# edshkim98/DiffusionIQT

Hardware: AMD Instinct MI355X
Metric: 3D patches/sec (32³, 1ch) — sample steps/sec x batch (one U-Net eval per patch and step: DDPM ancestral; EDM Heun in `edm` / `unet3d_edm`, train-steps/sec in `train`) (higher is better)
Workload: dtype f32; 1 GPU; C2: SRUnet256 dim=64 mults=(1,2,4) 32^3 1ch, batch 8/GPU, DDPM ancestral sampler step (1 U-Net eval = 186.06 GFLOP/patch); global_batch=8, patch=32^3, parallelism=dp1

## Files before the change

### diffusioniqt_amd/_lib.py

```python
import ctypes
import os

import torch
from ctypes import c_int, c_float, c_size_t, c_void_p, c_longlong, c_char_p

_HERE = os.path.dirname(os.path.abspath(__file__))
LIB_PATH = os.environ.get("DIQT_LIB") or os.path.join(_HERE, "csrc", "libdiqt_hip.so")

P, I, F, Z, L = c_void_p, c_int, c_float, c_size_t, c_longlong

PROTOTYPES = {
    "diqt_version": (I, []),
    "diqt_last_error": (c_char_p, []),
    "diqt_census_enable": (I, [I]),
    "diqt_census_count": (L, [c_char_p]),
    "diqt_get_last_launch": (c_char_p, []),
    "diqt_conv_packed_elems": (Z, [I, I, I, I, I]),
    "diqt_conv_packed_wino_elems": (Z, [I, I, I, I, I]),
    "diqt_conv_pack_weight": (I, [P, P, I, I, I, I, I, I, P]),
    "diqt_conv3d_fwd": (I, [P, P, P, P, P] + [I] * 15 + [P]),
    "diqt_conv3d_fwd_workspace_bytes": (Z, [I] * 15),
    "diqt_conv3d_fwd_ws": (I, [P, P, P, P, P, P, Z] + [I] * 15 + [P]),
    "diqt_conv3d_lds_bytes": (L, [I] * 12),
    "diqt_trilinear_up_fwd": (I, [P, P, I, I, I, I, I, I, P]),
# ... 198 lines not shown
    "diqt_conv_packed_split16_elems": (Z, [I, I, I, I, I]),
    "diqt_conv_pack_weight_split16": (I, [P, P, P, I, I, I, I, I, P]),
    "diqt_conv3d_fwd_split16_supported": (I, [I] * 15),
    "diqt_conv3d_fwd_gn_split16_supported": (I, [I] * 16),
    "diqt_conv3d_fwd_split16_stats_blocks": (I, [I] * 15),
    "diqt_conv3d_fwd_split16_variant": (I, [I] * 15),
    "diqt_conv3d_fwd_split16": (I, [P, P, P, P, P, P, P] + [I] * 15 + [P]),
    "diqt_conv3d_fwd_gn_split16": (I, [P, P, P, P, P, P, P, P, I] + [I] * 15 + [P]),
    "diqt_set_conv_split16_fill_tile": (I, [I]),
    "diqt_conv3d_fwd_split16_fill_supported": (I, [I] * 15),
    "diqt_conv3d_fwd_gn_split16_fill_supported": (I, [I] * 16),
    "diqt_conv3d_fwd_split16_fill_stats_blocks": (I, [I] * 15),
    "diqt_conv3d_fwd_split16_fill_variant": (I, [I] * 15),
    "diqt_conv3d_fwd_split16_fill": (I, [P, P, P, P, P, P, P] + [I] * 15 + [P]),
    "diqt_conv3d_fwd_gn_split16_fill": (I, [P, P, P, P, P, P, P, P, I] + [I] * 15 + [P]),
}

_lib = None


def load():
    global _lib
    if _lib is not None:
        return _lib
    if not os.path.exists(LIB_PATH):
        raise RuntimeError(
            f"diffusioniqt_amd: {LIB_PATH} is missing — build it with `python -c 'import __graft_entry__ as g; "
            f"g.build()'` or `bash diffusioniqt_amd/csrc/build.sh`. There is no CPU fallback.")
    lib = ctypes.CDLL(LIB_PATH)
    for name, (res, args) in PROTOTYPES.items():
# ... 75 lines not shown
```

### diffusioniqt_amd/csrc/conv_f9h_kernel.h

```cpp
#pragma once
#include "common.h"
#include "conv_f9h.h"

namespace diqt {
namespace h9 {

typedef float f32x16 __attribute__((ext_vector_type(16)));
typedef float f32x4v __attribute__((ext_vector_type(4)));
typedef unsigned u32x4 __attribute__((ext_vector_type(4)));
typedef unsigned u32x2 __attribute__((ext_vector_type(2)));
typedef _Float16 f16x8 __attribute__((ext_vector_type(8)));
typedef __bf16 bf16x8 __attribute__((ext_vector_type(8)));
typedef __attribute__((address_space(3))) void lds_void;

constexpr unsigned OOB = 0x80000000u;
constexpr int CK = 32, ROWB = 64;
constexpr int PD = 9;
constexpr int SCRW = 32 * 144;
constexpr int BIASB = 256;

#ifndef DIQT_F9H_STAMP
#define DIQT_F9H_STAMP(it, c, point)
#endif

// ... 495 lines not shown
    lds += BIASB;
    hipError_t e = hipFuncSetAttribute(reinterpret_cast<const void*>(kern), hipFuncAttributeMaxDynamicSharedMemorySize, (int)lds);
    DIQT_REQUIRE(e == hipSuccess, DIQT_E_LAUNCH, "conv3d_fwd_split16(v9h): hipFuncSetAttribute: %s", hipGetErrorString(e));
    hipLaunchKernelGGL(kern, dim3(grid), dim3(256), lds, (hipStream_t)stream, x, wp, bias, residual, y, g);
    return check_launch("conv3d_fwd_split16(v9h)");
}

int launch_b(const void* x, const unsigned short* wp, const float* bias, const float* residual, void* y, const H9Geom& g, size_t lds,
             unsigned grid, int bf16, bool yHalf, void* stream);
int launch_c(const void* x, const unsigned short* wp, const float* bias, const float* residual, void* y, const H9Geom& g, size_t lds,
             unsigned grid, int bf16, bool yHalf, void* stream);
int launch_split(const void* x, const unsigned short* wp, const float* bias, const float* residual, void* y, const H9Geom& g, size_t lds,
                 unsigned grid, void* stream);
int launch_split_b(const void* x, const unsigned short* wp, const float* bias, const float* residual, void* y, const H9Geom& g, size_t lds,
                   unsigned grid, void* stream);

}
}
```

### diffusioniqt_amd/csrc/conv_split16.hip

```cpp
#include "conv_f9h_kernel.h"
#include <atomic>

namespace diqt {

constexpr int S16_CG = 16;
constexpr float S16_MAX = 65504.f, S16_SCALE = 2048.f;

__device__ __forceinline__ float s16_clamp(float v) { return v > S16_MAX ? S16_MAX : (v < -S16_MAX ? -S16_MAX : v); }

__device__ __forceinline__ void s16_split(float v, _Float16& head, _Float16& tail) {
    head = (_Float16)s16_clamp(v);
    tail = (_Float16)s16_clamp((v - (float)head) * S16_SCALE);
}

__global__ __launch_bounds__(256) void conv_pack_weight_split16_kernel(const float* __restrict__ w, unsigned short* __restrict__ packed,
                                                                       int* __restrict__ refused, int Cout, int Cin, int T, int CoutPad,
                                                                       size_t total) {
    for (size_t i = blockIdx.x * (size_t)blockDim.x + threadIdx.x; i < total; i += (size_t)gridDim.x * blockDim.x) {
        const int k = (int)(i % h9::CK);
        size_t r = i / h9::CK;
        const int o = (int)(r % CoutPad);
        r /= CoutPad;
        const int tap = (int)(r % T);
        const int in = (int)(r / T) * S16_CG + (k & (S16_CG - 1));
// ... 31 lines not shown
            s16_split(v[e], h, t);
            head[e] = h; tail[e] = t;
        }
        unsigned short* row = y + vox * (size_t)(2 * C) + (size_t)(c8 >> 1) * 32u + (c8 & 1u) * 8u;
        *reinterpret_cast<h8*>(row) = head;
        *reinterpret_cast<h8*>(row + S16_CG) = tail;
    }
}

namespace h9 {

int launch_split(const void* x, const unsigned short* wp, const float* bias, const float* residual, void* y, const H9Geom& g, size_t lds,
                 unsigned grid, void* stream) {
    if (g.variant == 6) return launch_split_cfg<H9S_333_256>(x, wp, bias, residual, y, g, lds, grid, stream);
    if (g.variant == 7 || g.variant == 8) return launch_split_b(x, wp, bias, residual, y, g, lds, grid, stream);
    set_error("conv3d_fwd_split16(v9h): no variant %d", g.variant);
    return DIQT_E_UNSUPPORTED;
}

}
}

using namespace diqt;

extern "C" int diqt_set_conv_f9h_mode(int mode);

static bool split16_plan(H9Geom& g, size_t& lds, unsigned& grid, int B, int D, int H, int W, int Cin, int Cout, int kd, int kh, int kw, int pd,
                         int ph, int pw, int epd, int eph, int epw) {
    if (Cin <= 0 || Cin % S16_CG != 0 || Cin > (1 << 20)) return false;
    if (!f9h_plan(g, lds, grid, B, D, H, W, 2 * Cin, Cout, kd, kh, kw, pd, ph, pw, epd, eph, epw, false, true)) return false;
// ... 17 lines not shown
        if (forced && v != forced) continue;
        H9Geom t; size_t l; unsigned gr;
        if (!f9h_plan(t, l, gr, B, D, H, W, 2 * Cin, Cout, kd, kh, kw, pd, ph, pw, epd, eph, epw, false, true, v)) continue;
        g = t; lds = l; grid = gr; have = true;
        if ((long long)t.MT * t.nNt >= 256) break;
    }
    if (!have) return false;
    if (!lifted) {
        if ((long long)g.MT * g.nNt < 128) return false;
        if (g.variant == 8 && (long long)g.MT * g.nNt < 256 && Cin > 128) return false;
        if ((unsigned long long)B * g.Do * g.Ho * g.Wo * (unsigned long long)Cin * (unsigned long long)Cout < (1ull << 25)) return false;
    }
    return true;
}

static bool split16_any_plan(bool fill, H9Geom& g, size_t& lds, unsigned& grid, int B, int D, int H, int W, int Cin, int Cout, int kd, int kh,
                             int kw, int pd, int ph, int pw, int epd, int eph, int epw) {
    return fill ? split16_fill_plan(g, lds, grid, B, D, H, W, Cin, Cout, kd, kh, kw, pd, ph, pw, epd, eph, epw)
                : split16_plan(g, lds, grid, B, D, H, W, Cin, Cout, kd, kh, kw, pd, ph, pw, epd, eph, epw);
}

static bool split16_act_ok(int act) { return act == 0 || act == DIQT_ACT_MISH || act == DIQT_ACT_SILU || act == DIQT_ACT_GELU; }

extern "C" size_t diqt_conv_packed_split16_elems(int Cout, int Cin, int kd, int kh, int kw) {
    if (Cout <= 0 || Cin <= 0 || kd <= 0 || kh <= 0 || kw <= 0) return 0;
    return (size_t)((Cin + S16_CG - 1) / S16_CG) * kd * kh * kw * ((Cout + 63) / 64 * 64) * h9::CK;
}

extern "C" int diqt_conv_pack_weight_split16(const float* w, void* packed, int* refused, int Cout, int Cin, int kd, int kh, int kw,
                                             void* stream) {
    DIQT_REQUIRE(w && packed && refused, DIQT_E_ALIGN, "conv_pack_weight_split16: null pointer");
    DIQT_REQUIRE(Cout > 0 && Cin > 0 && kd > 0 && kh > 0 && kw > 0, DIQT_E_SHAPE, "conv_pack_weight_split16: bad shape");
    const int T = kd * kh * kw, CoutPad = (Cout + 63) / 64 * 64;
    const size_t total = diqt_conv_packed_split16_elems(Cout, Cin, kd, kh, kw);
// ... 17 lines not shown

extern "C" int diqt_conv3d_fwd_split16_stats_blocks(int B, int D, int H, int W, int Cin, int Cout, int kd, int kh, int kw, int pd, int ph,
                                                    int pw, int epd, int eph, int epw) {
    H9Geom g; size_t lds; unsigned grid;
    if (!split16_plan(g, lds, grid, B, D, H, W, Cin, Cout, kd, kh, kw, pd, ph, pw, epd, eph, epw)) return 0;
    return f9h_stats_blocks(g);
}

extern "C" int diqt_conv3d_fwd_split16_variant(int B, int D, int H, int W, int Cin, int Cout, int kd, int kh, int kw, int pd, int ph, int pw,
                                               int epd, int eph, int epw) {
    H9Geom g; size_t lds; unsigned grid;
    if (!split16_plan(g, lds, grid, B, D, H, W, Cin, Cout, kd, kh, kw, pd, ph, pw, epd, eph, epw)) return -1;
    return g.variant;
}

static int split16_run(const char* who, bool fill, const float* x, void* x16, const void* packed, const float* bias, const float* residual, float* y,
                       float* stats, const float* coef, int act, int B, int D, int H, int W, int Cin, int Cout, int kd, int kh, int kw, int pd,
                       int ph, int pw, int epd, int eph, int epw, void* stream) {
    DIQT_REQUIRE(x && x16 && packed && y, DIQT_E_ALIGN, "%s: null pointer", who);
    DIQT_REQUIRE(aligned16(x) && aligned16(x16) && aligned16(packed) && aligned16(y) && (!residual || aligned16(residual)) &&
                 (!coef || aligned16(coef)), DIQT_E_ALIGN, "%s: tensors must be 16-byte aligned", who);
    DIQT_REQUIRE(split16_act_ok(act), DIQT_E_UNSUPPORTED, "%s: activation %d", who, act);
    H9Geom g; size_t lds; unsigned grid;
    DIQT_REQUIRE(split16_any_plan(fill, g, lds, grid, B, D, H, W, Cin, Cout, kd, kh, kw, pd, ph, pw, epd, eph, epw), DIQT_E_UNSUPPORTED,
                 "%s: shape not taken by the split route (diqt_conv3d_fwd_split16%s_supported == 0)", who, fill ? "_fill" : "");
    const unsigned rows = (unsigned)D * H * W;
    const size_t total8 = (size_t)B * rows * (Cin / 8);
    if (coef)
        hipLaunchKernelGGL(split16_act_kernel<true>, dim3(grid_for(total8, 256)), dim3(256), 0, (hipStream_t)stream, x, coef, act,
                           static_cast<unsigned short*>(x16), B, rows, Cin, total8);
    else
        hipLaunchKernelGGL(split16_act_kernel<false>, dim3(grid_for(total8, 256)), dim3(256), 0, (hipStream_t)stream, x, coef, 0,
                           static_cast<unsigned short*>(x16), B, rows, Cin, total8);
    const int rc = check_launch("split16_act");
    if (rc != DIQT_OK) return rc;
    g.stats = stats;
    return f9h_launch_split(x16, static_cast<const unsigned short*>(packed), bias, residual, y, g, lds, grid, stream);
}

extern "C" int diqt_conv3d_fwd_split16(const float* x, void* x16, const void* packed, const float* bias, const float* residual, float* y,
                                       float* stats, int B, int D, int H, int W, int Cin, int Cout, int kd, int kh, int kw, int pd, int ph,
                                       int pw, int epd, int eph, int epw, void* stream) {
    return split16_run("conv3d_fwd_split16", false, x, x16, packed, bias, residual, y, stats, nullptr, 0, B, D, H, W, Cin, Cout, kd, kh, kw, pd, ph, pw,
                       epd, eph, epw, stream);
}

extern "C" int diqt_conv3d_fwd_gn_split16(const float* x, void* x16, const void* packed, const float* bias, const float* residual, float* y,
                                          float* stats, const float* coef, int act, int B, int D, int H, int W, int Cin, int Cout, int kd,
                                          int kh, int kw, int pd, int ph, int pw, int epd, int eph, int epw, void* stream) {
    DIQT_REQUIRE(coef, DIQT_E_ALIGN, "conv3d_fwd_gn_split16: null coefficients");
    return split16_run("conv3d_fwd_gn_split16", false, x, x16, packed, bias, residual, y, stats, coef, act, B, D, H, W, Cin, Cout, kd, kh, kw, pd, ph, pw,
                       epd, eph, epw, stream);
}

extern "C" int diqt_conv3d_fwd_split16_fill_supported(int B, int D, int H, int W, int Cin, int Cout, int kd, int kh, int kw, int pd, int ph,
                                                      int pw, int epd, int eph, int epw) {
    H9Geom g; size_t lds; unsigned grid;
    return split16_fill_plan(g, lds, grid, B, D, H, W, Cin, Cout, kd, kh, kw, pd, ph, pw, epd, eph, epw) ? 1 : 0;
}

extern "C" int diqt_conv3d_fwd_gn_split16_fill_supported(int B, int D, int H, int W, int Cin, int Cout, int kd, int kh, int kw, int pd, int ph,
                                                         int pw, int epd, int eph, int epw, int act) {
    return split16_act_ok(act) ? diqt_conv3d_fwd_split16_fill_supported(B, D, H, W, Cin, Cout, kd, kh, kw, pd, ph, pw, epd, eph, epw) : 0;
}

extern "C" int diqt_conv3d_fwd_split16_fill_stats_blocks(int B, int D, int H, int W, int Cin, int Cout, int kd, int kh, int kw, int pd, int ph,
// ... 1 lines not shown
    H9Geom g; size_t lds; unsigned grid;
    if (!split16_fill_plan(g, lds, grid, B, D, H, W, Cin, Cout, kd, kh, kw, pd, ph, pw, epd, eph, epw)) return 0;
    return f9h_stats_blocks(g);
}

extern "C" int diqt_conv3d_fwd_split16_fill_variant(int B, int D, int H, int W, int Cin, int Cout, int kd, int kh, int kw, int pd, int ph,
                                                    int pw, int epd, int eph, int epw) {
    H9Geom g; size_t lds; unsigned grid;
    if (!split16_fill_plan(g, lds, grid, B, D, H, W, Cin, Cout, kd, kh, kw, pd, ph, pw, epd, eph, epw)) return -1;
    return g.variant;
}

extern "C" int diqt_conv3d_fwd_split16_fill(const float* x, void* x16, const void* packed, const float* bias, const float* residual, float* y,
                                            float* stats, int B, int D, int H, int W, int Cin, int Cout, int kd, int kh, int kw, int pd,
                                            int ph, int pw, int epd, int eph, int epw, void* stream) {
    return split16_run("conv3d_fwd_split16_fill", true, x, x16, packed, bias, residual, y, stats, nullptr, 0, B, D, H, W, Cin, Cout, kd, kh, kw,
                       pd, ph, pw, epd, eph, epw, stream);
}

extern "C" int diqt_conv3d_fwd_gn_split16_fill(const float* x, void* x16, const void* packed, const float* bias, const float* residual,
                                               float* y, float* stats, const float* coef, int act, int B, int D, int H, int W, int Cin,
                                               int Cout, int kd, int kh, int kw, int pd, int ph, int pw, int epd, int eph, int epw,
                                               void* stream) {
    DIQT_REQUIRE(coef, DIQT_E_ALIGN, "conv3d_fwd_gn_split16_fill: null coefficients");
    return split16_run("conv3d_fwd_gn_split16_fill", true, x, x16, packed, bias, residual, y, stats, coef, act, B, D, H, W, Cin, Cout, kd, kh,
                       kw, pd, ph, pw, epd, eph, epw, stream);
}
```

### diffusioniqt_amd/imagen_pytorch3D.py

```python
import math
from contextlib import contextmanager, nullcontext
from functools import partial
from pathlib import Path

import numpy as np
import torch
import torch.nn.functional as F
from torch import nn

from . import ops
from .ops import ACT_MISH, ACT_GELU



def exists(val):
    return val is not None


def default(val, d):
    if exists(val):
        return val
    return d() if callable(d) else d


# ... 259 lines not shown

class LearnedSinusoidalPosEmb(nn.Module):
    def __init__(self, dim):
        super().__init__()
        assert (dim % 2) == 0
        self.weights = nn.Parameter(torch.randn(dim // 2))

    def forward(self, x):
        return ops.learned_sinusoidal(x, self.weights)


def _split16_pays(x, weight):
    if torch.is_grad_enabled() or ops.lp_mode() is not None or x.dim() != 5 or tuple(weight.shape[2:]) != (3, 3, 3):
        return False
    geo = (*x.shape, weight.shape[0], 3, 3, 3, 1, 1, 1, 0, 0, 0)
    if ops._lib.query("diqt_conv3d_fwd_split16_fill_supported", *geo):
        return "fill"
    return bool(ops._lib.query("diqt_conv3d_fwd_split16_supported", *geo))


def boundary_pad(x, batch_sample_factor=3):
    A = x.shape[1]
    vol = ops.merge_volume(x, batch_sample_factor)
    return ops.split_volume(vol, batch_sample_factor, A, halo=1)


class Block(nn.Module):

    def __init__(self, dim, dim_out, groups=8, norm=True, boundary=False, factor=3):
        super().__init__()
# ... 1394 lines not shown
```

### diffusioniqt_amd/ops.py

```python
import contextlib
import os

import torch
from torch.autograd import Function

from . import _lib

ACT_NONE, ACT_MISH, ACT_SILU, ACT_GELU, ACT_RELU, ACT_SIGMOID = range(6)

_WEIGHT_EPOCH = 0


def bump_weight_epoch():
    global _WEIGHT_EPOCH
    _WEIGHT_EPOCH += 1
    if _LIVE_GRAPHS > 0:
        from . import graphs
        graphs.drop_all()


_GRAPH_PINS = []
_LIVE_GRAPHS = 0


# ... 204 lines not shown
    Cout, Cin, kd, kh, kw = weight5.shape
    n = _lib.query("diqt_conv_packed_split16_elems", Cout, Cin, kd, kh, kw)
    packed = torch.empty(n, dtype=torch.int16, device=weight5.device)
    refused = torch.empty(1, dtype=torch.int32, device=weight5.device)
    _lib.call("diqt_conv_pack_weight_split16", weight5.detach(), packed, refused, Cout, Cin, kd, kh, kw, _stream())
    if hit is not None:
        retire(hit[1])
    packed = None if int(refused.item()) else born(packed)
    cache[slot] = (key, packed)
    return packed


def _split16_plan(geo, act, split16):
    if not split16 or not SPLIT16:
        return None
    if split16 == "fill" and _lib.query("diqt_conv3d_fwd_gn_split16_fill_supported", *geo, act):
        return "_fill"
    return "" if _lib.query("diqt_conv3d_fwd_gn_split16_supported", *geo, act) else None


def _conv_fwd_split16(x5, weight, bias, residual, pad, epad, want_stats, coef=None, act=0, split16=True):
    B, D, H, W, Cin = x5.shape
    Cout, _, kd, kh, kw = weight.shape
    geo = (B, D, H, W, Cin, Cout, kd, kh, kw, *pad, *epad)
    plan = _split16_plan(geo, act, split16)
    if plan is None:
        return None
    packed = _packed_split16(weight)
    if packed is None:
        return None
    Do, Ho, Wo = D + 2 * pad[0] + epad[0] - kd + 1, H + 2 * pad[1] + epad[1] - kh + 1, W + 2 * pad[2] + epad[2] - kw + 1
# ... 3228 lines not shown
```

### include/diqt.h

```cpp
#ifndef DIQT_H
#define DIQT_H

#include <stddef.h>
#include <stdint.h>

#ifdef __cplusplus
extern "C" {
#endif

#define DIQT_OK             0
#define DIQT_E_SHAPE       -1
#define DIQT_E_ALIGN       -2
#define DIQT_E_UNSUPPORTED -3
#define DIQT_E_LAUNCH      -4
#define DIQT_E_WORKSPACE   -5

#define DIQT_ACT_NONE    0
#define DIQT_ACT_MISH    1
#define DIQT_ACT_SILU    2
#define DIQT_ACT_GELU    3
#define DIQT_ACT_RELU    4
#define DIQT_ACT_SIGMOID 5

int         diqt_version(void);
// ... 56 lines not shown
int diqt_set_conv_split16_fill_tile(int variant);
int diqt_conv3d_fwd_split16_fill_supported(int B, int D, int H, int W, int Cin, int Cout, int kd, int kh, int kw, int pd, int ph, int pw,
                                           int epd, int eph, int epw);
int diqt_conv3d_fwd_gn_split16_fill_supported(int B, int D, int H, int W, int Cin, int Cout, int kd, int kh, int kw, int pd, int ph, int pw,
                                              int epd, int eph, int epw, int act);
int diqt_conv3d_fwd_split16_fill_stats_blocks(int B, int D, int H, int W, int Cin, int Cout, int kd, int kh, int kw, int pd, int ph, int pw,
                                              int epd, int eph, int epw);
int diqt_conv3d_fwd_split16_fill_variant(int B, int D, int H, int W, int Cin, int Cout, int kd, int kh, int kw, int pd, int ph, int pw,
                                         int epd, int eph, int epw);
int diqt_conv3d_fwd_split16_fill(const float* x, void* x16, const void* packed, const float* bias, const float* residual, float* y,
                                 float* stats, int B, int D, int H, int W, int Cin, int Cout, int kd, int kh, int kw, int pd, int ph, int pw,
                                 int epd, int eph, int epw, void* stream);
int diqt_conv3d_fwd_gn_split16_fill(const float* x, void* x16, const void* packed, const float* bias, const float* residual, float* y,
                                    float* stats, const float* coef, int act, int B, int D, int H, int W, int Cin, int Cout, int kd, int kh,
                                    int kw, int pd, int ph, int pw, int epd, int eph, int epw, void* stream);

int diqt_conv3d_fwd_kernel_id(int B, int D, int H, int W, int Cin, int Cout, int kd, int kh, int kw, int pd, int ph, int pw,
                              int epd, int eph, int epw);
int diqt_conv3d_fwd9_variant(int B, int D, int H, int W, int Cin, int Cout, int kd, int kh, int kw, int pd, int ph, int pw,
                             int epd, int eph, int epw, size_t packed_elems);
int diqt_conv3d_fwd_route(int B, int D, int H, int W, int Cin, int Cout, int kd, int kh, int kw, int pd, int ph, int pw,
                          int epd, int eph, int epw, size_t packed_elems, int has_workspace, int has_stats, int sub_f, int gn_act,
                          int field);
int diqt_get_last_conv_fwd9_variant(void);
int diqt_conv3d_fwd_stats_blocks(int B, int D, int H, int W, int Cin, int Cout, int kd, int kh, int kw, int pd, int ph, int pw,
                                 int epd, int eph, int epw);
int diqt_conv3d_fwd_ex(const float* x, const float* packed, const float* bias, const float* residual, float* y, float* stats,
                       void* workspace, size_t workspace_bytes, int B, int D, int H, int W, int Cin, int Cout,
                       int kd, int kh, int kw, int pd, int ph, int pw, int epd, int eph, int epw, void* stream);
int diqt_conv3d_fwd_pk(const float* x, const float* packed, size_t packed_elems, const float* bias, const float* residual, float* y,
// ... 411 lines not shown
```

Before: 1438 patches/s.

## Add paired-tap split16 3x3x3 conv kernel using 16x16x32 f16 MFMA

Adds a new split16 conv kernel variant that packs two filter taps per K step, so it can use the v_mfma_f32_16x16x32_f16 instruction over 14 steps instead of a per-tap schedule. It uses a swizzled LDS layout with a compile-time bank-conflict checker, a 7-deep weight register ring, halo DMA spread across steps, and a head/tail split-precision accumulate in the epilogue. The Python dispatch now prefers this pair path when it is supported, falling back to fill and then plain split16. The cost is more register pressure (launch bounds of one block) and wasted MFMA work on the padded 28th tap.

```diff
diff --git a/diffusioniqt_amd/_lib.py b/diffusioniqt_amd/_lib.py
--- a/diffusioniqt_amd/_lib.py
+++ b/diffusioniqt_amd/_lib.py
@@ -236,6 +236,12 @@
     "diqt_conv3d_fwd_split16_fill_variant": (I, [I] * 15),
     "diqt_conv3d_fwd_split16_fill": (I, [P, P, P, P, P, P, P] + [I] * 15 + [P]),
     "diqt_conv3d_fwd_gn_split16_fill": (I, [P, P, P, P, P, P, P, P, I] + [I] * 15 + [P]),
+    "diqt_conv3d_fwd_split16_pair_supported": (I, [I] * 15),
+    "diqt_conv3d_fwd_gn_split16_pair_supported": (I, [I] * 16),
+    "diqt_conv3d_fwd_split16_pair_stats_blocks": (I, [I] * 15),
+    "diqt_conv3d_fwd_split16_pair": (I, [P, P, P, P, P, P, P] + [I] * 15 + [P]),
+    "diqt_conv3d_fwd_gn_split16_pair": (I, [P, P, P, P, P, P, P, P, I] + [I] * 15 + [P]),
+    "diqt_conv_split16_pair_lds_conflicts": (I, []),
 }
 
 _lib = None
diff --git a/diffusioniqt_amd/csrc/conv_f9h_kernel.h b/diffusioniqt_amd/csrc/conv_f9h_kernel.h
--- a/diffusioniqt_amd/csrc/conv_f9h_kernel.h
+++ b/diffusioniqt_amd/csrc/conv_f9h_kernel.h
@@ -533,6 +533,8 @@
                  unsigned grid, void* stream);
 int launch_split_b(const void* x, const unsigned short* wp, const float* bias, const float* residual, void* y, const H9Geom& g, size_t lds,
                    unsigned grid, void* stream);
-
-}
-}
+int launch_split_c(const void* x, const unsigned short* wp, const float* bias, const float* residual, void* y, const H9Geom& g, size_t lds,
+                   unsigned grid, void* stream);
+
+}
+}
diff --git a/diffusioniqt_amd/csrc/conv_f9p_kernel.h b/diffusioniqt_amd/csrc/conv_f9p_kernel.h
--- /dev/null
+++ b/diffusioniqt_amd/csrc/conv_f9p_kernel.h
@@ -0,0 +1,351 @@
+#pragma once
+#include "conv_f9h_kernel.h"
+
+namespace diqt {
+namespace h9 {
+
+constexpr int PAIR_STEPS = 14;
+
+__host__ __device__ constexpr int pair_col_j(int m, int h) { return h + 2 * (((m >> 2) ^ (m >> 3)) & 1); }
+__host__ __device__ constexpr int pair_col_i(int m) { return 4 * (m >> 3) + (m & 3); }
+__host__ __device__ constexpr int pair_col_row(int m, int h) {
+    const int t2 = ((m >> 2) ^ (m >> 3)) & 1, t1 = m >> 3;
+    return (t2 << 4) | (t1 << 3) | ((h ^ t1 ^ t2) << 2) | (m & 3);
+}
+__host__ __device__ constexpr int pair_tap(int p, int kg) { return 2 * p + (kg >> 1) < 27 ? 2 * p + (kg >> 1) : 26; }
+template <class C> __host__ __device__ constexpr int pair_lds_addr_t(int m, int ko, int t, int h, int q, int wa) {
+    const int ky = (t / C::KW) % C::KH, kx = t % C::KW;
+    const int j = pair_col_j(m, h), i = pair_col_i(m);
+    const int gx = ((i + kx) >> 2) & 1, gy = ((j + ky) >> 1) & 1;
+    return (C::blockrow(0) + (wa ? C::blockrow(C::NVB) : 0) + j * C::HWd + i + C::tapoff(t)) * ROWB + ((ko ^ gx) << 4) + ((q ^ gy) << 5);
+}
+template <class C> __host__ __device__ constexpr int pair_lds_addr(int l, int p, int h, int q, int wa) {
+    const int a0 = pair_lds_addr_t<C>(l & 15, (l >> 4) & 1, pair_tap(p, 0), h, q, wa), a1 = pair_lds_addr_t<C>(l & 15, (l >> 4) & 1, pair_tap(p, 2), h, q, wa);
+    return (l >> 5) ? a1 : a0;
+}
+__host__ __device__ constexpr int b128_group_lane(int s, int e) {
+    const int in32 = (s & 1) ? (e < 8 ? 4 + e : (e < 12 ? 8 + e : 16 + e)) : (e < 4 ? e : (e < 8 ? 8 + e : 12 + e));
+    return 32 * (s >> 1) + in32;
+}
+template <class C> constexpr int pair_lds_conflicts() {
+    int worst = 0;
+    for (int wa = 0; wa < 2; ++wa)
+        for (int p = 0; p < PAIR_STEPS; ++p)
+            for (int cb = 0; cb < 2 * C::NVB; ++cb)
+                for (int q = 0; q < 2; ++q)
+                    for (int s = 0; s < 4; ++s) {
+                        int addr[16] = {};
+                        for (int e = 0; e < 16; ++e)
+                            addr[e] = pair_lds_addr<C>(b128_group_lane(s, e), p, cb & 1, q, wa) + (C::blockrow(cb >> 1) - C::blockrow(0)) * ROWB;
+                        for (int e = 0; e < 16; ++e) {
+                            int n = 0;
+                            for (int f = 0; f < 16; ++f) {
+                                if (((addr[f] >> 4) & 15) != ((addr[e] >> 4) & 15)) continue;
+                                bool seen = false;
+                                for (int k = 0; k < f; ++k) seen = seen || addr[k] == addr[f];
+                                if (!seen) ++n;
+                            }
+                            if (n > worst) worst = n;
+                        }
+                    }
+    return worst;
+}
+
+template <bool Z> __device__ __forceinline__ void mfma_pair(f32x4v& c, const u32x4& a, const u32x4& b) {
+    if (Z) asm volatile("v_mfma_f32_16x16x32_f16 %0, %1, %2, 0" : "=a"(c) : "v"(a), "v"(b));
+    else asm volatile("v_mfma_f32_16x16x32_f16 %0, %1, %2, %0" : "+a"(c) : "v"(a), "v"(b));
+}
+
+template <class C, int RS, int PD>
+__global__ __launch_bounds__(256, 1) void conv_f9p_kernel(const void* __restrict__ xv, const unsigned short* __restrict__ wp,
+                                                          const float* __restrict__ bias, const float* __restrict__ residual,
+                                                          void* __restrict__ yv, H9Geom g) {
+    constexpr int T = C::T, HB = C::HB, NPH = C::NPH, NVB = C::NVB, HH = C::HH, HWd = C::HWd, HV = C::HV, NIMG = C::NIMG;
+    constexpr int NS = PAIR_STEPS, NCB = 2 * NVB;
+    static_assert(T == 27 && NIMG == 2 && NVB == 4, "the pair body is written for the 3x3x3 filter on the 256-voxel tile");
+    static_assert(NS % PD == 0 && PD >= 2, "the ring slot of a step is static");
+    constexpr int NSP = NS - PD + 1;
+    static_assert(NSP >= 1, "halo pieces need a step to ride on");
+    extern __shared__ __attribute__((aligned(1024))) char smem[];
+    const int tid = threadIdx.x, lane = tid & 63, wave = __builtin_amdgcn_readfirstlane(tid >> 6);
+    const int m = lane & 15, kg = lane >> 4;
+    const int wa = wave >> 1, wb = wave & 1;
+    const unsigned Gn = gridDim.x;
+    const unsigned total = (unsigned)g.MT * g.nNt;
+    unsigned L = xcd_remap(blockIdx.x, Gn);
+    if (L >= total) return;
+    DIQT_F9H_STAMP(0, 0, 7);
+    const unsigned L0 = L;
+    const int nMine = (int)((total - 1 - L) / Gn) + 1;
+    const int n0 = (int)(L % g.nNt) * 64;
+    const int nChunks = g.nChunks;
+
+    const auto rs_x = __builtin_amdgcn_make_buffer_rsrc(const_cast<void*>(xv), 0, (int)g.xBytes, 0x00020000);
+    const auto rs_w = __builtin_amdgcn_make_buffer_rsrc(const_cast<unsigned short*>(wp), 0, (int)g.wBytes, 0x00020000);
+    const auto rs_y = __builtin_amdgcn_make_buffer_rsrc(yv, 0, (int)g.yBytes, 0x00020000);
+    const auto rs_r = __builtin_amdgcn_make_buffer_rsrc(const_cast<float*>(residual), 0, residual ? (int)g.rBytes : 0, 0x00020000);
+    const unsigned ldsBase = (unsigned)(size_t)(lds_void*)smem;
+
+    unsigned posH[NPH];
+#pragma unroll
+    for (int r = 0; r < NPH; ++r) {
+        const int p = (wave + 4 * r) * 64 + lane;
+        const int row = p >> 2;
+        const int hx = row % HWd, hy = (row / HWd) % HH, hz = row / (HWd * HH);
+        const int gsw = ((hx >> 2) & 1) | (((hy >> 1) & 1) << 1);
+        posH[r] = (unsigned)hz | ((unsigned)hy << 10) | ((unsigned)(row < HV ? hx : 1023) << 20) | ((unsigned)((p & 3) ^ gsw) << 30);
+    }
+    const int Dm1 = g.D - 1, Hm1 = g.H - 1, Wm1 = g.W - 1;
+    int tb, d0, h0, w0;
+    int bz = 0, by = 0, bxx = 0;
+    unsigned baseX = 0, deadX = OOB;
+    auto tile_of = [&](unsigned Lt, int& b_, int& d_, int& h_, int& w_) __attribute__((always_inline)) {
+        int mt = (int)(Lt / g.nNt);
+        const int tx = mt % g.tilesW; mt /= g.tilesW;
+        const int ty = mt % g.tilesH; mt /= g.tilesH;
+        const int tz = mt % g.tilesD;
+        b_ = mt / g.tilesD; d_ = tz * C::TD; h_ = ty * C::TH; w_ = tx * C::TW;
+    };
+    auto set_fetch = [&](int fit_) __attribute__((always_inline)) {
+        const bool live = fit_ < nMine;
+        int b_, d_, h_, w_;
+        tile_of(live ? L0 + (unsigned)fit_ * Gn : L0, b_, d_, h_, w_);
+        bz = d_ - g.pd; by = h_ - g.ph; bxx = w_ - g.pw;
+        baseX = (unsigned)((((b_ * g.D + bz) * g.H + by) * g.W + bxx) * g.Cin) * 2u;
+        deadX = live ? 0u : OOB;
+    };
+    const int HWs = g.W * g.Cin * 2, HHs = g.H * HWs, Cs = g.Cin * 2;
+    auto dma_h = [&](int r, unsigned imgBase, int chunk) __attribute__((always_inline)) {
+        const unsigned p = posH[r];
+        const int hz = (int)(p & 1023u), hy = (int)((p >> 10) & 1023u), hx = (int)((p >> 20) & 1023u);
+        const int iz = bz + hz, iy = by + hy, ix = bxx + hx;
+        const unsigned mk = (unsigned)(iz | iy | ix) | (unsigned)((Dm1 - iz) | (Hm1 - iy) | (Wm1 - ix)) | deadX;
+        const unsigned rel = (unsigned)(hz * HHs + hy * HWs + hx * Cs) + ((p >> 30) << 4);
+        const unsigned voff = (baseX + rel + (unsigned)chunk * ROWB) | (mk & OOB);
+        dma16(rs_x, imgBase + (unsigned)(wave + 4 * r) * 1024u, voff);
+    };
+
+    const unsigned wStride = (unsigned)g.CoutPad * ROWB;
+    const unsigned wLane = (unsigned)((n0 + 32 * wb + m) * ROWB + (kg & 1) * 16) + (unsigned)(kg >> 1) * wStride;
+    const unsigned wLane13 = (kg >> 1) ? OOB : wLane;
+    const int WT = nChunks * T;
+    u32x4 Wr[PD][2][2];
+    int wlin = 0;
+    unsigned wsoff = 0;
+    auto w_load = [&](int slot, bool last) __attribute__((always_inline)) {
+        const unsigned vo = last ? wLane13 : wLane;
+#pragma unroll
+        for (int rb = 0; rb < 2; ++rb) {
+            Wr[slot][rb][0] = __builtin_amdgcn_raw_buffer_load_b128(rs_w, vo + (unsigned)rb * 16u * ROWB, wsoff, 0);
+            Wr[slot][rb][1] = __builtin_amdgcn_raw_buffer_load_b128(rs_w, vo + (unsigned)rb * 16u * ROWB + 32u, wsoff, 0);
+        }
+        wsoff += last ? wStride : 2u * wStride;
+        wlin += last ? 1 : 2;
+        if (wlin == WT) { wlin = 0; wsoff = 0; }
+    };
+
+    int xa[NS][2][2];
+#pragma unroll
+    for (int p = 0; p < NS; ++p)
+#pragma unroll
+        for (int h = 0; h < 2; ++h)
+#pragma unroll
+            for (int q = 0; q < 2; ++q) xa[p][h][q] = pair_lds_addr<C>(lane, p, h, q, wa);
+
+    const auto rs_b = __builtin_amdgcn_make_buffer_rsrc(const_cast<float*>(bias), 0, bias ? g.Cout * 4 : 0, 0x00020000);
+    f32x4v acc[2][NCB], acc1[2][NCB];
+
+    int fit = 0, fc = 0;
+    set_fetch(0);
+    auto advance_fetch = [&]() __attribute__((always_inline)) {
+        if (++fc == nChunks) { fc = 0; ++fit; set_fetch(fit); }
+    };
+#pragma unroll
+    for (int r = 0; r < NPH; ++r) dma_h(r, ldsBase, fc);
+    advance_fetch();
+#pragma unroll
+    for (int s = 0; s < PD - 1; ++s) w_load(s, false);
+    if (tid < 64)
+        reinterpret_cast<float*>(smem + C::LDS_BYTES)[tid] =
+            __builtin_bit_cast(float, __builtin_amdgcn_raw_buffer_load_b32(rs_b, (unsigned)(n0 + tid) * 4u, 0, 0));
+    __builtin_amdgcn_s_waitcnt(0x0f70);
+    __syncthreads();
+
+    int img = 0, fimg = 1;
+    tile_of(L, tb, d0, h0, w0);
+    for (int it = 0; it < nMine; ++it) {
+#pragma unroll
+        for (int pass = 0; pass < 2; ++pass)
+        for (int c = pass; c < (pass == 0 ? 1 : nChunks); ++c) {
+            const bool FIRST = pass == 0;
+            const unsigned fbase = ldsBase + (unsigned)fimg * HB;
+            const int delta = (img ? -1 : 1) * HB;
+            u32x4 Xh[2][NCB], Xl[2][NCB];
+            auto rd = [&](int p, int cb, int q) __attribute__((always_inline)) {
+                const u32x4 v = *reinterpret_cast<const u32x4*>(smem + xa[p][cb & 1][q] + (C::blockrow(cb >> 1) - C::blockrow(0)) * ROWB);
+                if (q) Xl[p & 1][cb] = v; else Xh[p & 1][cb] = v;
+            };
+            DIQT_F9H_STAMP(it, c, 0);
+#pragma unroll
+            for (int cb = 0; cb < NCB; ++cb) { rd(0, cb, 0); rd(0, cb, 1); }
+#pragma unroll
+            for (int p = 0; p < NS; ++p) {
+                __builtin_amdgcn_sched_barrier(0);
+                const int s = p % PD, cur = p & 1;
+                const bool Z = FIRST && p == 0;
+#pragma unroll
+                for (int cb = 0; cb < NCB; ++cb) {
+                    if (p + 1 < NS) rd(p + 1, cb, 0);
+                    if (Z) {
+                        mfma_pair<true>(acc1[0][cb], Wr[s][0][1], Xh[cur][cb]);
+                        mfma_pair<true>(acc1[1][cb], Wr[s][1][1], Xh[cur][cb]);
+                        mfma_pair<true>(acc[0][cb], Wr[s][0][0], Xh[cur][cb]);
+                    } else {
+                        mfma_pair<false>(acc1[0][cb], Wr[s][0][1], Xh[cur][cb]);
+                        mfma_pair<false>(acc1[1][cb], Wr[s][1][1], Xh[cur][cb]);
+                        mfma_pair<false>(acc[0][cb], Wr[s][0][0], Xh[cur][cb]);
+                    }
+                    __builtin_amdgcn_sched_barrier(0);
+                    if (p + 1 < NS) rd(p + 1, cb, 1);
+                    if (Z) mfma_pair<true>(acc[1][cb], Wr[s][1][0], Xh[cur][cb]);
+                    else mfma_pair<false>(acc[1][cb], Wr[s][1][0], Xh[cur][cb]);
+                    mfma_pair<false>(acc1[0][cb], Wr[s][0][0], Xl[cur][cb]);
+                    mfma_pair<false>(acc1[1][cb], Wr[s][1][0], Xl[cur][cb]);
+                    if (cb == 1) {
+#pragma unroll
+                        for (int r = 0; r < NPH; ++r)
+                            if (r * NSP / NPH == p) dma_h(r, fbase, fc);
+                    }
+                    if (cb == 3) w_load((p + PD - 1) % PD, (p + PD - 1) % NS == NS - 1);
+                    if (cb >= NCB - 2) { const int pn = (p + 1) % NS; xa[pn][cb & 1][0] += delta; xa[pn][cb & 1][1] += delta; }
+                    __builtin_amdgcn_sched_barrier(0);
+                }
+                if (p == PD - 2) { DIQT_F9H_STAMP(it, c, 1); }
+            }
+            DIQT_F9H_STAMP(it, c, 2);
+            asm volatile("s_barrier" ::: "memory");
+            DIQT_F9H_STAMP(it, c, 3);
+            advance_fetch();
+            {
+                fimg = img;
+                img ^= 1;
+            }
+        }
+        asm volatile("s_nop 15\n\ts_nop 15");
+        {
+            constexpr int SROW = 144;
+            const bool hasRes = (RS & 1) != 0;
+            const bool wantStats = (RS & 2) != 0;
+            char* const scrb = smem + fimg * HB + wave * SCRW;
+            const int piece = lane & 7, vl = lane >> 3;
+            const int cop = n0 + 32 * wb + piece * 4;
+            const bool cok = cop < g.Cout;
+            const unsigned C4 = (unsigned)g.Cout * 4u;
+            int rjk[4], rik[4];
+            unsigned lo[4];
+#pragma unroll
+            for (int k = 0; k < 4; ++k) {
+                const int vloc = 8 * k + vl, tqr = vloc >> 2;
+                rjk[k] = 2 * (tqr >> 2) + ((tqr ^ (tqr >> 1) ^ (tqr >> 2)) & 1);
+                rik[k] = 4 * (k & 1) + (vl & 3);
+                lo[k] = cok ? (unsigned)(rjk[k] * g.Wo + rik[k]) * C4 + (unsigned)cop * 4u : OOB;
+            }
+            const unsigned tileOff = (unsigned)(((tb * g.Do + d0) * g.Ho + h0) * g.Wo + w0) * C4;
+            auto offs = [&](int vb, unsigned (&vo)[4], unsigned& so) __attribute__((always_inline)) {
+                const int id = wa * NVB + vb;
+                const int bd = id / (C::NBH * C::NBW), bh = ((id / C::NBW) % C::NBH) * 4, bw = (id % C::NBW) * 8;
+                so = tileOff + (unsigned)((bd * g.Ho + bh) * g.Wo + bw) * C4;
+                const int hlim = d0 + bd < g.Do ? g.Ho - h0 - bh : 0, wlim = g.Wo - w0 - bw;
+#pragma unroll
+                for (int k = 0; k < 4; ++k) vo[k] = ((int)(rjk[k] < hlim) & (int)(rik[k] < wlim)) ? lo[k] : OOB;
+            };
+            float ssum[4], ssq[4];
+#pragma unroll
+            for (int e = 0; e < 4; ++e) { ssum[e] = 0.f; ssq[e] = 0.f; }
+            f32x4v b4[2];
+#pragma unroll
+            for (int rb = 0; rb < 2; ++rb)
+                b4[rb] = *reinterpret_cast<const f32x4v*>(smem + C::LDS_BYTES + (32 * wb + 16 * rb + 4 * kg) * 4);
+            const int srow0 = pair_col_row(m, 0) * SROW, srow1 = pair_col_row(m, 1) * SROW;
+            unsigned vo[2][4], so[2];
+            f32x4v rr[2][4];
+            offs(0, vo[0], so[0]);
+            if (hasRes) {
+#pragma unroll
+                for (int k = 0; k < 4; ++k) rr[0][k] = __builtin_bit_cast(f32x4v, __builtin_amdgcn_raw_buffer_load_b128(rs_r, vo[0][k], so[0], 0));
+            }
+            DIQT_F9H_STAMP(it, 0, 4);
+#pragma unroll
+            for (int vb = 0; vb < NVB; ++vb) {
+                const int cur = vb & 1, nxt = cur ^ 1;
+#pragma unroll
+                for (int h = 0; h < 2; ++h)
+#pragma unroll
+                    for (int rb = 0; rb < 2; ++rb) {
+                        f32x4v p;
+#pragma unroll
+                        for (int e = 0; e < 4; ++e) p[e] = fmaf(acc1[rb][2 * vb + h][e], 0x1p-11f, acc[rb][2 * vb + h][e]) + b4[rb][e];
+                        *reinterpret_cast<f32x4v*>(scrb + (h ? srow1 : srow0) + 64 * rb + 16 * kg) = p;
+                    }
+                if (vb + 1 < NVB) {
+                    offs(vb + 1, vo[nxt], so[nxt]);
+                    if (hasRes) {
+#pragma unroll
+                        for (int k = 0; k < 4; ++k)
+                            rr[nxt][k] = __builtin_bit_cast(f32x4v, __builtin_amdgcn_raw_buffer_load_b128(rs_r, vo[nxt][k], so[nxt], 0));
+                    }
+                }
+                u32x4 d[4];
+#pragma unroll
+                for (int k = 0; k < 4; ++k) d[k] = *reinterpret_cast<const u32x4*>(scrb + (8 * k + vl) * SROW + piece * 16);
+#pragma unroll
+                for (int k = 0; k < 4; ++k) {
+                    if (hasRes) {
+                        f32x4v f = __builtin_bit_cast(f32x4v, d[k]);
+#pragma unroll
+                        for (int e = 0; e < 4; ++e) f[e] += rr[cur][k][e];
+                        d[k] = __builtin_bit_cast(u32x4, f);
+                    }
+                    if (wantStats) {
+                        const float okf = vo[cur][k] != OOB ? 1.f : 0.f;
+#pragma unroll
+                        for (int e = 0; e < 4; ++e) {
+                            const unsigned wd = d[k][e];
+                            const float v = __builtin_bit_cast(float, wd);
+                            const float mv = okf * v;
+                            ssum[e] += mv;
+                            ssq[e] = fmaf(mv, v, ssq[e]);
+                        }
+                    }
+                    __builtin_amdgcn_raw_buffer_store_b128(d[k], rs_y, vo[cur][k], so[cur], 0);
+                }
+            }
+            DIQT_F9H_STAMP(it, 0, 5);
+            if (wantStats) {
+                const int tpb = g.tilesD * g.tilesH * g.tilesW, mtile = (int)(L / g.nNt);
+                float* srow = g.stats + ((size_t)(mtile / tpb) * (2 * tpb) + (size_t)(mtile % tpb) * 2 + wa) * 2 * g.Cout;
+#pragma unroll
+                for (int e = 0; e < 4; ++e) {
+#pragma unroll
+                    for (int o = 8; o < 64; o <<= 1) {
+                        ssum[e] += __shfl_xor(ssum[e], o, 64);
+                        ssq[e] += __shfl_xor(ssq[e], o, 64);
+                    }
+                }
+                if (lane < 8 && cok) {
+#pragma unroll
+                    for (int e = 0; e < 4; ++e) { srow[cop + e] = ssum[e]; srow[g.Cout + cop + e] = ssq[e]; }
+                }
+            }
+        }
+        asm volatile("s_barrier" ::: "memory");
+        DIQT_F9H_STAMP(it, 0, 6);
+        L += Gn;
+        if (it + 1 < nMine) tile_of(L, tb, d0, h0, w0);
+    }
+    __builtin_amdgcn_s_waitcnt(0x0f70);
+    DIQT_F9H_STAMP(0, 0, 8);
+}
+
+}
+}
diff --git a/diffusioniqt_amd/csrc/conv_split16.hip b/diffusioniqt_amd/csrc/conv_split16.hip
--- a/diffusioniqt_amd/csrc/conv_split16.hip
+++ b/diffusioniqt_amd/csrc/conv_split16.hip
@@ -69,6 +69,7 @@
                  unsigned grid, void* stream) {
     if (g.variant == 6) return launch_split_cfg<H9S_333_256>(x, wp, bias, residual, y, g, lds, grid, stream);
     if (g.variant == 7 || g.variant == 8) return launch_split_b(x, wp, bias, residual, y, g, lds, grid, stream);
+    if (g.variant == 9) return launch_split_c(x, wp, bias, residual, y, g, lds, grid, stream);
     set_error("conv3d_fwd_split16(v9h): no variant %d", g.variant);
     return DIQT_E_UNSUPPORTED;
 }
@@ -116,10 +117,28 @@
     return true;
 }
 
-static bool split16_any_plan(bool fill, H9Geom& g, size_t& lds, unsigned& grid, int B, int D, int H, int W, int Cin, int Cout, int kd, int kh,
+static bool split16_pair_plan(H9Geom& g, size_t& lds, unsigned& grid, int B, int D, int H, int W, int Cin, int Cout, int kd, int kh, int kw,
+                              int pd, int ph, int pw, int epd, int eph, int epw) {
+    if (Cin <= 0 || Cin % S16_CG != 0 || Cin > (1 << 20)) return false;
+    if (!f9h_plan(g, lds, grid, B, D, H, W, 2 * Cin, Cout, kd, kh, kw, pd, ph, pw, epd, eph, epw, false, true, 6)) return false;
+    if (diqt_set_conv_f9h_mode(-1) != 2) {
+        const long long units = (long long)g.MT * g.nNt;
+        if (units < 256) return false;
+        if ((unsigned long long)B * g.Do * g.Ho * g.Wo * (unsigned long long)Cin * (unsigned long long)Cout < (1ull << 25)) return false;
+        if (units <= (long long)grid && g.nChunks < 8) return false;
+    }
+    g.variant = 9;
+    return true;
+}
+
+enum { S16_PLAN = 0, S16_FILL = 1, S16_PAIR = 2 };
+static const char* const s16_suffix[3] = {"", "_fill", "_pair"};
+
+static bool split16_any_plan(int plan, H9Geom& g, size_t& lds, unsigned& grid, int B, int D, int H, int W, int Cin, int Cout, int kd, int kh,
                              int kw, int pd, int ph, int pw, int epd, int eph, int epw) {
-    return fill ? split16_fill_plan(g, lds, grid, B, D, H, W, Cin, Cout, kd, kh, kw, pd, ph, pw, epd, eph, epw)
-                : split16_plan(g, lds, grid, B, D, H, W, Cin, Cout, kd, kh, kw, pd, ph, pw, epd, eph, epw);
+    if (plan == S16_PAIR) return split16_pair_plan(g, lds, grid, B, D, H, W, Cin, Cout, kd, kh, kw, pd, ph, pw, epd, eph, epw);
+    return plan == S16_FILL ? split16_fill_plan(g, lds, grid, B, D, H, W, Cin, Cout, kd, kh, kw, pd, ph, pw, epd, eph, epw)
+                            : split16_plan(g, lds, grid, B, D, H, W, Cin, Cout, kd, kh, kw, pd, ph, pw, epd, eph, epw);
 }
 
 static bool split16_act_ok(int act) { return act == 0 || act == DIQT_ACT_MISH || act == DIQT_ACT_SILU || act == DIQT_ACT_GELU; }
@@ -167,7 +186,7 @@
     return g.variant;
 }
 
-static int split16_run(const char* who, bool fill, const float* x, void* x16, const void* packed, const float* bias, const float* residual, float* y,
+static int split16_run(const char* who, int plan, const float* x, void* x16, const void* packed, const float* bias, const float* residual, float* y,
                        float* stats, const float* coef, int act, int B, int D, int H, int W, int Cin, int Cout, int kd, int kh, int kw, int pd,
                        int ph, int pw, int epd, int eph, int epw, void* stream) {
     DIQT_REQUIRE(x && x16 && packed && y, DIQT_E_ALIGN, "%s: null pointer", who);
@@ -175,8 +194,8 @@
                  (!coef || aligned16(coef)), DIQT_E_ALIGN, "%s: tensors must be 16-byte aligned", who);
     DIQT_REQUIRE(split16_act_ok(act), DIQT_E_UNSUPPORTED, "%s: activation %d", who, act);
     H9Geom g; size_t lds; unsigned grid;
-    DIQT_REQUIRE(split16_any_plan(fill, g, lds, grid, B, D, H, W, Cin, Cout, kd, kh, kw, pd, ph, pw, epd, eph, epw), DIQT_E_UNSUPPORTED,
-                 "%s: shape not taken by the split route (diqt_conv3d_fwd_split16%s_supported == 0)", who, fill ? "_fill" : "");
+    DIQT_REQUIRE(split16_any_plan(plan, g, lds, grid, B, D, H, W, Cin, Cout, kd, kh, kw, pd, ph, pw, epd, eph, epw), DIQT_E_UNSUPPORTED,
+                 "%s: shape not taken by the split route (diqt_conv3d_fwd_split16%s_supported == 0)", who, s16_suffix[plan]);
     const unsigned rows = (unsigned)D * H * W;
     const size_t total8 = (size_t)B * rows * (Cin / 8);
     if (coef)
@@ -194,7 +213,7 @@
 extern "C" int diqt_conv3d_fwd_split16(const float* x, void* x16, const void* packed, const float* bias, const float* residual, float* y,
                                        float* stats, int B, int D, int H, int W, int Cin, int Cout, int kd, int kh, int kw, int pd, int ph,
                                        int pw, int epd, int eph, int epw, void* stream) {
-    return split16_run("conv3d_fwd_split16", false, x, x16, packed, bias, residual, y, stats, nullptr, 0, B, D, H, W, Cin, Cout, kd, kh, kw, pd, ph, pw,
+    return split16_run("conv3d_fwd_split16", S16_PLAN, x, x16, packed, bias, residual, y, stats, nullptr, 0, B, D, H, W, Cin, Cout, kd, kh, kw, pd, ph, pw,
                        epd, eph, epw, stream);
 }
 
@@ -202,7 +221,7 @@
                                           float* stats, const float* coef, int act, int B, int D, int H, int W, int Cin, int Cout, int kd,
                                           int kh, int kw, int pd, int ph, int pw, int epd, int eph, int epw, void* stream) {
     DIQT_REQUIRE(coef, DIQT_E_ALIGN, "conv3d_fwd_gn_split16: null coefficients");
-    return split16_run("conv3d_fwd_gn_split16", false, x, x16, packed, bias, residual, y, stats, coef, act, B, D, H, W, Cin, Cout, kd, kh, kw, pd, ph, pw,
+    return split16_run("conv3d_fwd_gn_split16", S16_PLAN, x, x16, packed, bias, residual, y, stats, coef, act, B, D, H, W, Cin, Cout, kd, kh, kw, pd, ph, pw,
                        epd, eph, epw, stream);
 }
 
@@ -234,7 +253,7 @@
 extern "C" int diqt_conv3d_fwd_split16_fill(const float* x, void* x16, const void* packed, const float* bias, const float* residual, float* y,
                                             float* stats, int B, int D, int H, int W, int Cin, int Cout, int kd, int kh, int kw, int pd,
                                             int ph, int pw, int epd, int eph, int epw, void* stream) {
-    return split16_run("conv3d_fwd_split16_fill", true, x, x16, packed, bias, residual, y, stats, nullptr, 0, B, D, H, W, Cin, Cout, kd, kh, kw,
+    return split16_run("conv3d_fwd_split16_fill", S16_FILL, x, x16, packed, bias, residual, y, stats, nullptr, 0, B, D, H, W, Cin, Cout, kd, kh, kw,
                        pd, ph, pw, epd, eph, epw, stream);
 }
 
@@ -243,6 +262,40 @@
                                                int Cout, int kd, int kh, int kw, int pd, int ph, int pw, int epd, int eph, int epw,
                                                void* stream) {
     DIQT_REQUIRE(coef, DIQT_E_ALIGN, "conv3d_fwd_gn_split16_fill: null coefficients");
-    return split16_run("conv3d_fwd_gn_split16_fill", true, x, x16, packed, bias, residual, y, stats, coef, act, B, D, H, W, Cin, Cout, kd, kh,
+    return split16_run("conv3d_fwd_gn_split16_fill", S16_FILL, x, x16, packed, bias, residual, y, stats, coef, act, B, D, H, W, Cin, Cout, kd, kh,
                        kw, pd, ph, pw, epd, eph, epw, stream);
 }
+
+extern "C" int diqt_conv3d_fwd_split16_pair_supported(int B, int D, int H, int W, int Cin, int Cout, int kd, int kh, int kw, int pd, int ph,
+                                                      int pw, int epd, int eph, int epw) {
+    H9Geom g; size_t lds; unsigned grid;
+    return split16_pair_plan(g, lds, grid, B, D, H, W, Cin, Cout, kd, kh, kw, pd, ph, pw, epd, eph, epw) ? 1 : 0;
+}
+
+extern "C" int diqt_conv3d_fwd_gn_split16_pair_supported(int B, int D, int H, int W, int Cin, int Cout, int kd, int kh, int kw, int pd, int ph,
+                                                         int pw, int epd, int eph, int epw, int act) {
+    return split16_act_ok(act) ? diqt_conv3d_fwd_split16_pair_supported(B, D, H, W, Cin, Cout, kd, kh, kw, pd, ph, pw, epd, eph, epw) : 0;
+}
+
+extern "C" int diqt_conv3d_fwd_split16_pair_stats_blocks(int B, int D, int H, int W, int Cin, int Cout, int kd, int kh, int kw, int pd, int ph,
+                                                         int pw, int epd, int eph, int epw) {
+    H9Geom g; size_t lds; unsigned grid;
+    if (!split16_pair_plan(g, lds, grid, B, D, H, W, Cin, Cout, kd, kh, kw, pd, ph, pw, epd, eph, epw)) return 0;
+    return f9h_stats_blocks(g);
+}
+
+extern "C" int diqt_conv3d_fwd_split16_pair(const float* x, void* x16, const void* packed, const float* bias, const float* residual, float* y,
+                                            float* stats, int B, int D, int H, int W, int Cin, int Cout, int kd, int kh, int kw, int pd,
+                                            int ph, int pw, int epd, int eph, int epw, void* stream) {
+    return split16_run("conv3d_fwd_split16_pair", S16_PAIR, x, x16, packed, bias, residual, y, stats, nullptr, 0, B, D, H, W, Cin, Cout, kd, kh,
+                       kw, pd, ph, pw, epd, eph, epw, stream);
+}
+
+extern "C" int diqt_conv3d_fwd_gn_split16_pair(const float* x, void* x16, const void* packed, const float* bias, const float* residual,
+                                               float* y, float* stats, const float* coef, int act, int B, int D, int H, int W, int Cin,
+                                               int Cout, int kd, int kh, int kw, int pd, int ph, int pw, int epd, int eph, int epw,
+                                               void* stream) {
+    DIQT_REQUIRE(coef, DIQT_E_ALIGN, "conv3d_fwd_gn_split16_pair: null coefficients");
+    return split16_run("conv3d_fwd_gn_split16_pair", S16_PAIR, x, x16, packed, bias, residual, y, stats, coef, act, B, D, H, W, Cin, Cout, kd,
+                       kh, kw, pd, ph, pw, epd, eph, epw, stream);
+}
diff --git a/diffusioniqt_amd/csrc/conv_split16_c.hip b/diffusioniqt_amd/csrc/conv_split16_c.hip
--- /dev/null
+++ b/diffusioniqt_amd/csrc/conv_split16_c.hip
@@ -0,0 +1,30 @@
+#include "conv_f9p_kernel.h"
+
+namespace diqt {
+namespace h9 {
+
+constexpr int PAIR_PD = 7;
+
+int launch_split_c(const void* x, const unsigned short* wp, const float* bias, const float* residual, void* y, const H9Geom& g, size_t lds,
+                   unsigned grid, void* stream) {
+    using C = H9S_333_256;
+    static_assert(C::LDS_BYTES + BIASB <= 160 * 1024, "LDS budget with the staged bias");
+    if (g.variant != 9) {
+        set_error("conv3d_fwd_split16_pair(v9p): no variant %d", g.variant);
+        return DIQT_E_UNSUPPORTED;
+    }
+    typedef void (*KP)(const void*, const unsigned short*, const float*, const float*, void*, H9Geom);
+    static const KP kerns[4] = {conv_f9p_kernel<C, 0, PAIR_PD>, conv_f9p_kernel<C, 1, PAIR_PD>, conv_f9p_kernel<C, 2, PAIR_PD>,
+                                conv_f9p_kernel<C, 3, PAIR_PD>};
+    const KP kern = kerns[(residual ? 1 : 0) | (g.stats ? 2 : 0)];
+    lds += BIASB;
+    hipError_t e = hipFuncSetAttribute(reinterpret_cast<const void*>(kern), hipFuncAttributeMaxDynamicSharedMemorySize, (int)lds);
+    DIQT_REQUIRE(e == hipSuccess, DIQT_E_LAUNCH, "conv3d_fwd_split16_pair(v9p): hipFuncSetAttribute: %s", hipGetErrorString(e));
+    hipLaunchKernelGGL(kern, dim3(grid), dim3(256), lds, (hipStream_t)stream, x, wp, bias, residual, y, g);
+    return check_launch("conv3d_fwd_split16(v9h)");
+}
+
+}
+}
+
+extern "C" int diqt_conv_split16_pair_lds_conflicts(void) { return diqt::h9::pair_lds_conflicts<diqt::h9::H9S_333_256>(); }
diff --git a/diffusioniqt_amd/imagen_pytorch3D.py b/diffusioniqt_amd/imagen_pytorch3D.py
--- a/diffusioniqt_amd/imagen_pytorch3D.py
+++ b/diffusioniqt_amd/imagen_pytorch3D.py
@@ -297,6 +297,8 @@
     if torch.is_grad_enabled() or ops.lp_mode() is not None or x.dim() != 5 or tuple(weight.shape[2:]) != (3, 3, 3):
         return False
     geo = (*x.shape, weight.shape[0], 3, 3, 3, 1, 1, 1, 0, 0, 0)
+    if ops._lib.query("diqt_conv3d_fwd_split16_pair_supported", *geo):
+        return "pair"
     if ops._lib.query("diqt_conv3d_fwd_split16_fill_supported", *geo):
         return "fill"
     return bool(ops._lib.query("diqt_conv3d_fwd_split16_supported", *geo))
diff --git a/diffusioniqt_amd/ops.py b/diffusioniqt_amd/ops.py
--- a/diffusioniqt_amd/ops.py
+++ b/diffusioniqt_amd/ops.py
@@ -242,7 +242,9 @@
 def _split16_plan(geo, act, split16):
     if not split16 or not SPLIT16:
         return None
-    if split16 == "fill" and _lib.query("diqt_conv3d_fwd_gn_split16_fill_supported", *geo, act):
+    if split16 == "pair" and _lib.query("diqt_conv3d_fwd_gn_split16_pair_supported", *geo, act):
+        return "_pair"
+    if split16 in ("fill", "pair") and _lib.query("diqt_conv3d_fwd_gn_split16_fill_supported", *geo, act):
         return "_fill"
     return "" if _lib.query("diqt_conv3d_fwd_gn_split16_supported", *geo, act) else None
 
diff --git a/include/diqt.h b/include/diqt.h
--- a/include/diqt.h
+++ b/include/diqt.h
@@ -94,6 +94,19 @@
 int diqt_conv3d_fwd_gn_split16_fill(const float* x, void* x16, const void* packed, const float* bias, const float* residual, float* y,
                                     float* stats, const float* coef, int act, int B, int D, int H, int W, int Cin, int Cout, int kd, int kh,
                                     int kw, int pd, int ph, int pw, int epd, int eph, int epw, void* stream);
+int diqt_conv3d_fwd_split16_pair_supported(int B, int D, int H, int W, int Cin, int Cout, int kd, int kh, int kw, int pd, int ph, int pw,
+                                           int epd, int eph, int epw);
+int diqt_conv3d_fwd_gn_split16_pair_supported(int B, int D, int H, int W, int Cin, int Cout, int kd, int kh, int kw, int pd, int ph, int pw,
+                                              int epd, int eph, int epw, int act);
+int diqt_conv3d_fwd_split16_pair_stats_blocks(int B, int D, int H, int W, int Cin, int Cout, int kd, int kh, int kw, int pd, int ph, int pw,
+                                              int epd, int eph, int epw);
+int diqt_conv3d_fwd_split16_pair(const float* x, void* x16, const void* packed, const float* bias, const float* residual, float* y,
+                                 float* stats, int B, int D, int H, int W, int Cin, int Cout, int kd, int kh, int kw, int pd, int ph, int pw,
+                                 int epd, int eph, int epw, void* stream);
+int diqt_conv3d_fwd_gn_split16_pair(const float* x, void* x16, const void* packed, const float* bias, const float* residual, float* y,
+                                    float* stats, const float* coef, int act, int B, int D, int H, int W, int Cin, int Cout, int kd, int kh,
+                                    int kw, int pd, int ph, int pw, int epd, int eph, int epw, void* stream);
+int diqt_conv_split16_pair_lds_conflicts(void);
 
 int diqt_conv3d_fwd_kernel_id(int B, int D, int H, int W, int Cin, int Cout, int kd, int kh, int kw, int pd, int ph, int pw,
                               int epd, int eph, int epw);
```

New measurement: 1492 patches/s (median of 6 runs). 3.7% higher.
